# PaullyMac/routest

Measured on AMD Instinct MI355X. Metric: ETA preds/sec (whole node) + p50 /predict latency, 3-layer MLP bf16, higher is better.
Workload: dtype bf16

## Files before the change

### csrc/cch_bindings.cpp

```cpp
#include <torch/extension.h>
#include <ATen/hip/impl/HIPStreamMasqueradingAsCUDA.h>
#include <c10/core/DeviceGuard.h>

#include <chrono>
#include <cmath>
#include <memory>
#include <mutex>
#include <unordered_map>

#include "cch_gpu.h"
#include "ops.h"

namespace py = pybind11;

namespace {

#define CCH_CHECK_HIP(expr)                                                            \
  do {                                                                                 \
    hipError_t _e = (expr);                                                            \
    TORCH_CHECK(_e == hipSuccess, "HIP error in ", #expr, ": ", hipGetErrorString(_e)); \
  } while (0)

hipStream_t stream_of(int dev) { return c10::hip::getCurrentHIPStreamMasqueradingAsCUDA(dev).stream(); }

// ... 123 lines not shown
    d["async_pending"] = a.pending;
    d["async_build_ms"] = a.build_ms;
    d["async_alloc_ms"] = a.alloc_ms;
    d["async_hostcopy_ms"] = a.hostcopy_ms;
    d["builder_max_wg"] = g_->builder_pacing();
    d["async_paced"] = a.paced;
    return d;
  }

  void request_build(int64_t weather, int64_t congestion, int64_t weekhour, double age, bool urgent,
                     c10::optional<torch::Tensor> avoid, int64_t avoid_digest) {
    TORCH_CHECK(g_->has_eta(), "CchGpu: set_eta first");
    const rt::CchContext c = context(weather, congestion, weekhour, age, avoid, avoid_digest);
    g_->request_build(c, urgent);
  }
  bool is_cached(int64_t key) {
    std::shared_ptr<rt::CchMetricDev> m;
    return g_->cached_metric((uint64_t)key, m);
  }
  void set_cache_gb(double gb) { g_->set_cache_gb(gb); }
  void set_builder_pacing(int n, bool always) { g_->set_builder_pacing(n, always); }
  void set_unpack_serial(bool on) { g_->set_unpack_serial(on); }
  bool unpack_serial() const { return g_->unpack_serial(); }

  py::dict info(const rt::CchMetricDev& m, bool fresh) const {
    py::dict d;
    d["key"] = m.key;
    d["fresh"] = fresh;
    d["cost_ms"] = m.cost_ms;
    d["customize_ms"] = m.customize_ms;
    d["basic_ms"] = m.basic_ms;
    d["perfect_ms"] = m.perfect_ms;
    d["prune_ms"] = m.prune_ms;
    d["kept_f"] = m.kept_f;
    d["kept_b"] = m.kept_b;
    return d;
  }

  py::dict metric_for(int64_t weather, int64_t congestion, int64_t weekhour, double age, bool pin,
                      c10::optional<torch::Tensor> avoid, int64_t avoid_digest) {
    TORCH_CHECK(g_->has_eta(), "CchGpu: set_eta first");
    const rt::CchContext c = context(weather, congestion, weekhour, age, avoid, avoid_digest);
    const c10::DeviceGuard guard(c10::Device(c10::DeviceType::CUDA, dev_));
    std::shared_ptr<rt::CchMetricDev> m;
    bool fresh = false;
    hipError_t e;
// ... 98 lines not shown
    o.path = want_path ? path.data_ptr<int>() : nullptr;
    o.max_path = (int)max_path;
    const c10::DeviceGuard guard(src.device());
    std::lock_guard<std::mutex> lk(mu_);
    CCH_CHECK_HIP(g_->route(*m, src.data_ptr<int>(), dst.data_ptr<int>(), (int)Q, o, *sc_, stream_of(dev_)));
    return py::make_tuple(sec, met, st, len, path);
  }

  py::tuple matrix(int64_t key, torch::Tensor pts, torch::Tensor npts) {
    auto m = get(key);
    TORCH_CHECK(pts.is_cuda() && npts.is_cuda() && pts.dim() == 2 && pts.scalar_type() == torch::kInt32 &&
                    npts.scalar_type() == torch::kInt32 && npts.numel() == pts.size(0) && pts.is_contiguous(),
                "pts int32 [R, NM], npts int32 [R] on the router's GPU");
    const int R = (int)pts.size(0), NM = (int)pts.size(1);
    auto of = torch::TensorOptions().dtype(torch::kFloat32).device(torch::kCUDA, dev_);
    auto sec = torch::empty({R, NM, NM}, of), met = torch::empty({R, NM, NM}, of);
    const c10::DeviceGuard guard(pts.device());
    std::lock_guard<std::mutex> lk(mu_);
    CCH_CHECK_HIP(g_->matrix(*m, pts.data_ptr<int>(), npts.data_ptr<int>(), R, NM, sec.data_ptr<float>(),
                             met.data_ptr<float>(), nullptr, *sc_, stream_of(dev_)));
    return py::make_tuple(sec, met);
  }

  py::tuple matrix_rect(int64_t key, torch::Tensor src, torch::Tensor nsrc, torch::Tensor dst, torch::Tensor ndst,
                        int64_t meet) {
    auto m = get(key);
    for (const torch::Tensor* t : {&src, &nsrc, &dst, &ndst})
      TORCH_CHECK(t->is_cuda() && t->device().index() == dev_ && t->scalar_type() == torch::kInt32 && t->is_contiguous(),
                  "src / nsrc / dst / ndst: int32 on the router's GPU");
    TORCH_CHECK(src.dim() == 2 && dst.dim() == 2 && dst.size(0) == src.size(0) && nsrc.numel() == src.size(0) &&
                    ndst.numel() == src.size(0),
                "src [R, SM], dst [R, DM], nsrc [R], ndst [R]");
    const int64_t R = src.size(0), SM = src.size(1), DM = dst.size(1);
    TORCH_CHECK(R * (SM + DM) <= INT32_MAX && R * SM * DM <= INT32_MAX, "matrix_rect: too many chains or cells for one call");
    auto of = torch::TensorOptions().dtype(torch::kFloat32).device(torch::kCUDA, dev_);
    auto sec = torch::empty({R, SM, DM}, of), met = torch::empty({R, SM, DM}, of);
    const c10::DeviceGuard guard(src.device());
    std::lock_guard<std::mutex> lk(mu_);
    CCH_CHECK_HIP(g_->matrix_rect(*m, src.data_ptr<int>(), nsrc.data_ptr<int>(), dst.data_ptr<int>(),
                                  ndst.data_ptr<int>(), (int)R, (int)SM, (int)DM, sec.data_ptr<float>(),
                                  met.data_ptr<float>(), *sc_, stream_of(dev_), (int)meet));
    return py::make_tuple(sec, met);
  }

  py::tuple matrix_keep(int64_t key, torch::Tensor pts, torch::Tensor npts) {
    auto sm = matrix(key, pts, npts);
// ... 107 lines not shown

}

void bind_cch_gpu(py::module& m) {
  py::class_<PyCchGpu>(m, "CchGpu")
      .def(py::init<torch::Tensor, torch::Tensor, torch::Tensor, torch::Tensor, torch::Tensor, torch::Tensor,
                    torch::Tensor, int64_t>(),
           py::arg("indptr"), py::arg("indices"), py::arg("lat"), py::arg("lon"), py::arg("length"),
           py::arg("road_class"), py::arg("base_traffic"), py::arg("device"))
      .def("set_eta", &PyCchGpu::set_eta, py::arg("blob"), py::arg("H"), py::arg("norm"), py::arg("variant") = -1)
      .def("stats", &PyCchGpu::stats)
      .def("metric_for", &PyCchGpu::metric_for, py::arg("weather"), py::arg("congestion"), py::arg("weekhour"),
           py::arg("driver_age") = 35.0, py::arg("pin") = false, py::arg("avoid") = py::none(),
           py::arg("avoid_digest") = 0)
      .def("avoid_mask", &PyCchGpu::avoid_mask, py::arg("blob"))
      .def("unpin", &PyCchGpu::unpin, py::arg("key"))
      .def("pinned", &PyCchGpu::pinned)
      .def("metric_from_costs", &PyCchGpu::metric_from_costs, py::arg("key"), py::arg("cost"))
      .def("costs", &PyCchGpu::costs, py::arg("key"))
      .def("metric_dump", &PyCchGpu::metric_dump, py::arg("key"))
      .def("route", &PyCchGpu::route, py::arg("key"), py::arg("src"), py::arg("dst"), py::arg("max_path") = 4096,
           py::arg("want_path") = true)
      .def("matrix", &PyCchGpu::matrix, py::arg("key"), py::arg("pts"), py::arg("npts"))
      .def("matrix_rect", &PyCchGpu::matrix_rect, py::arg("key"), py::arg("src"), py::arg("nsrc"), py::arg("dst"),
           py::arg("ndst"), py::arg("meet") = 0)
      .def("matrix_keep", &PyCchGpu::matrix_keep, py::arg("key"), py::arg("pts"), py::arg("npts"))
      .def("legs_from_matrix", &PyCchGpu::legs_from_matrix, py::arg("key"), py::arg("tag"), py::arg("pts"), py::arg("r"),
           py::arg("i"), py::arg("j"), py::arg("max_path") = 4096, py::arg("want_path") = true)
      .def("one_to_all", &PyCchGpu::one_to_all, py::arg("key"), py::arg("src"), py::arg("reverse") = false,
           py::arg("fuse") = -1)
      .def("set_capacity", &PyCchGpu::set_capacity)
      .def("set_cache_gb", &PyCchGpu::set_cache_gb, py::arg("gb"))
      .def("set_builder_pacing", &PyCchGpu::set_builder_pacing, py::arg("max_workgroups"), py::arg("always") = false)
      .def("set_unpack_serial", &PyCchGpu::set_unpack_serial, py::arg("on"))
      .def("unpack_serial", &PyCchGpu::unpack_serial)
      .def("request_build", &PyCchGpu::request_build, py::arg("weather"), py::arg("congestion"), py::arg("weekhour"),
           py::arg("driver_age") = 35.0, py::arg("urgent") = true, py::arg("avoid") = py::none(),
           py::arg("avoid_digest") = 0)
      .def("is_cached", &PyCchGpu::is_cached, py::arg("key"))
      .def("ptr", &PyCchGpu::ptr)
      .def("topology_arrays", &PyCchGpu::topology_arrays);
}
```

### csrc/cch_gpu.h

```cpp
#pragma once
#include <hip/hip_runtime.h>

#include <cstdint>
#include <cstdlib>
#include <cstring>
#include <atomic>
#include <chrono>
#include <condition_variable>
#include <deque>
#include <functional>
#include <list>
#include <memory>
#include <mutex>
#include <thread>
#include <unordered_set>
#include <vector>

#include "common.h"
#include "runtime/cch.h"

namespace rt {

struct CchContext {
  int weather = 2, congestion = 1, weekhour = 9;
// ... 15 lines not shown
  float* len_up = nullptr;
  float* len_dn = nullptr;
  int32_t* cnt_up = nullptr;
  int32_t* cnt_dn = nullptr;
  int32_t* f_ptr = nullptr;
  int32_t* b_ptr = nullptr;
  int4* f_rec = nullptr;
  int4* b_rec = nullptr;
  int64_t kept_f = 0, kept_b = 0;
  double customize_ms = 0.0, cost_ms = 0.0;
  double basic_ms = 0.0, perfect_ms = 0.0, prune_ms = 0.0;
  double alloc_ms = 0.0, hostcopy_ms = 0.0;
  std::vector<float> host_cost;
  std::shared_ptr<const std::vector<int32_t>> avoid;
  ~CchMetricDev();
};

struct CchScratch {
  float* dist = nullptr;
  int32_t* pred = nullptr;
  int32_t* node = nullptr;
  size_t jobs_cap = 0;
  int32_t* jobs = nullptr;
  int32_t* arcs = nullptr;
  int32_t* narcs = nullptr;
  size_t pairs_cap = 0;
  int32_t* pj = nullptr;
  size_t pj_cap = 0;
  uint64_t chain_tag = 0;
  int chain_nm = 0, chain_r = 0;
  int device = 0;
  std::vector<void*> old;
  ~CchScratch();
  hipError_t ensure(size_t jobs, size_t pairs, int stride, int max_arcs);
};

struct CchAllScratch {
  float* sec = nullptr;
  float* met = nullptr;
  size_t blocks_cap = 0;
  int device = 0;
  std::vector<void*> old;
  ~CchAllScratch();
  hipError_t ensure(size_t blocks, size_t N);
};

// ... 75 lines not shown
  double cache_gb() { std::lock_guard<std::mutex> lk(mu_); return cache_gb_; }
  int capacity() { std::lock_guard<std::mutex> lk(mu_); return capacity_; }
  int64_t metric_bytes() const { return metric_bytes_.load(); }
  int cached() { std::lock_guard<std::mutex> lk(mu_); return (int)cache_.size(); }

  void request_build(const CchContext& c, bool urgent = true);
  void start_builders();
  int add_build_listener(std::function<void(uint64_t, bool)> cb);
  void remove_build_listener(int id);
  struct AsyncStats {
    long long queued = 0, built = 0, failed = 0;
    int pending = 0;
    double build_ms = 0.0, alloc_ms = 0.0, hostcopy_ms = 0.0;
    long long paced = 0;
  };
  AsyncStats async_stats();
  void set_builder_pacing(int n, bool always = false) {
    builder_max_wg_.store(n < 0 ? 0 : n);
    pace_always_.store(always);
  }
  int builder_pacing() const { return builder_max_wg_.load(); }
  void set_unpack_serial(bool on) { unpack_serial_.store(on); }
  bool unpack_serial() const { return unpack_serial_.load(); }
  void note_queries() {
    query_us_.store(std::chrono::duration_cast<std::chrono::microseconds>(
                        std::chrono::steady_clock::now().time_since_epoch()).count(),
                    std::memory_order_relaxed);
  }
  bool serving_now() const {
    const long long now = std::chrono::duration_cast<std::chrono::microseconds>(
                              std::chrono::steady_clock::now().time_since_epoch()).count();
    return now - query_us_.load(std::memory_order_relaxed) < 250000;
  }

  hipError_t route(const CchMetricDev& m, const int* d_src, const int* d_dst, int Q, const CchRouteOut& o,
                   CchScratch& sc, hipStream_t s);
  hipError_t matrix(const CchMetricDev& m, const int* d_pts, const int* d_npts, int R, int NM, float* d_sec,
                    float* d_met, double* d_D64, CchScratch& sc, hipStream_t s);
  hipError_t legs_from_matrix(const CchMetricDev& m, const int* d_src, const int* d_r, const int* d_i, const int* d_j,
                              int Q, uint64_t tag, const CchRouteOut& o, CchScratch& sc, hipStream_t s);
  static constexpr int MAX_ARCS = 1024;
  enum { MEET_AUTO = 0, MEET_RECT = 1, MEET_PAIRS = 2, MEET_NONE = 3 };
  hipError_t matrix_rect(const CchMetricDev& m, const int* d_src, const int* d_nsrc, const int* d_dst,
                         const int* d_ndst, int R, int SM, int DM, float* d_sec, float* d_met, CchScratch& sc,
                         hipStream_t s, int meet = MEET_AUTO);

// ... 1 lines not shown
                        CchAllScratch& sc, hipStream_t s, int fuse = -1);
  static constexpr size_t ALL_SCRATCH_BYTES = 1ull << 30;
  static constexpr int ALL_FUSE_WIDTH = 4;

  static CchMView view(const CchMetricDev& m) {
    return CchMView{m.f_ptr, m.b_ptr, m.f_rec, m.b_rec, m.len_up, m.len_dn, m.sub_up, m.sub_dn, m.cnt_up, m.cnt_dn};
  }
  hipError_t route_multi(const CchMView* d_mv, const int* d_grp, const int* d_src, const int* d_dst, int Q,
                         const CchRouteOut& o, CchScratch& sc, hipStream_t s);
  hipError_t matrix_multi(const CchMView* d_mv, const int* d_row_grp, const int* d_pts, const int* d_npts, int R, int NM,
                          float* d_sec, float* d_met, double* d_D64, CchScratch& sc, hipStream_t s);
  hipError_t legs_from_matrix_multi(const CchMView* d_mv, const int* d_grp, const int* d_src, const int* d_r,
                                    const int* d_i, const int* d_j, int Q, uint64_t tag, const CchRouteOut& o,
                                    CchScratch& sc, hipStream_t s);

 private:
  hipError_t route_impl(const CchMetricDev* m, const CchMView* mv, const int* grp, const int* d_src, const int* d_dst,
                        int Q, const CchRouteOut& o, CchScratch& sc, hipStream_t s);
  hipError_t matrix_impl(const CchMetricDev* m, const CchMView* mv, const int* grp, const int* d_pts, const int* d_npts,
                         int R, int NM, float* d_sec, float* d_met, double* d_D64, CchScratch& sc, hipStream_t s);
  hipError_t legs_impl(const CchMetricDev* m, const CchMView* mv, const int* grp, const int* d_src, const int* d_r,
                       const int* d_i, const int* d_j, int Q, uint64_t tag, const CchRouteOut& o, CchScratch& sc,
                       hipStream_t s);
  hipError_t launch_unpack(const CchMetricDev* m, const CchMView* mv, const int* grp, int Q, const int* d_src,
                           CchScratch& sc, const CchRouteOut& o, hipStream_t s);
  rcch::Topology T_;
  int dev_ = 0;
  int32_t *d_up_ptr = nullptr, *d_up_head = nullptr, *d_arc_lo = nullptr, *d_parent = nullptr, *d_depth = nullptr;
  int32_t *d_rank = nullptr, *d_node = nullptr, *d_edge_arc = nullptr;
  uint8_t* d_edge_dir = nullptr;
  float* d_length = nullptr;
  uint8_t *d_class = nullptr, *d_base_traffic = nullptr;
  int32_t *d_hnodes = nullptr, *d_dnodes = nullptr;
  int32_t* d_dlev_ptr = nullptr;
  int64_t *d_bofs = nullptr, *d_pofs = nullptr;
  std::vector<int64_t> bofs_, pofs_, aofs_;
  std::vector<int> plev_kmax_;
  bool accel_ = false;
  void build_tables();
  void free_tables();
  bool build_triangles(const std::vector<int64_t>& tofs);
  int32_t* d_tri = nullptr;
  int64_t n_tri = 0;
  bool build_tasks(const std::vector<int64_t>& tofs);
  bool build_pull_records(const std::vector<int64_t>& tofs);
  void* d_btask = nullptr;
// ... 51 lines not shown
  int32_t *d_esrc = nullptr, *d_edst = nullptr, *d_qx = nullptr, *d_qy = nullptr;
  std::atomic<uint64_t> tag_ctr_{0};
  void builder_loop(int idx);
  void start_builders_locked();
  void notify_built(uint64_t key, bool ok);
  std::vector<std::thread> bths_;
  std::mutex bmu_;
  std::condition_variable bcv_;
  std::deque<CchContext> bq_;
  std::unordered_set<uint64_t> bpending_;
  bool bstop_ = false;
  std::mutex lmu_;
  std::vector<std::pair<int, std::function<void(uint64_t, bool)>>> listeners_;
  int next_listener_ = 1;
  std::atomic<long long> n_bqueued_{0}, n_bbuilt_{0}, n_bfailed_{0};
  std::atomic<long long> us_build_{0}, us_alloc_{0}, us_hostcopy_{0};
  std::atomic<long long> query_us_{-(1LL << 40)};
  std::atomic<bool> pace_always_{false};
  std::atomic<long long> n_paced_{0};
  std::atomic<int> builder_max_wg_{[] {
    const char* v = std::getenv("ROUTEST_CCH_BUILDER_MAX_WG");
    return v ? std::max(0, std::atoi(v)) : -1;
  }()};
  std::atomic<bool> unpack_serial_{[] {
    const char* v = std::getenv("ROUTEST_CCH_UNPACK");
    return v != nullptr && std::strcmp(v, "serial") == 0;
  }()};
};

}
```

### csrc/cch_query.hip

```cpp
#include "cch_dev.h"
#include "cch_gpu.h"

namespace rt {

using namespace cchd;

namespace {

constexpr int SWEEP_AHEAD = 3;
constexpr int SWEEP_RECS = 4;

typedef int sweep_v4i __attribute__((ext_vector_type(4)));

struct SweepRecs {
  sweep_v4i r[SWEEP_RECS];
};

__device__ __forceinline__ SweepRecs sweep_fetch(const int4* __restrict__ rec, int pb, int pe, int i, int L, int lane) {
  SweepRecs v;
  const int ii = i < 63 ? i : 63;
  const int b = __shfl(pb, ii);
  const int e = i < L ? __shfl(pe, ii) : b;
#pragma unroll
  for (int k = 0; k < SWEEP_RECS; ++k) {
    const int idx = b + lane + 64 * k;
    const int4* p = rec + (idx < e ? idx : 0);
    asm volatile("global_load_dwordx4 %0, %1, off" : "=v"(v.r[k]) : "v"(p));
  }
  return v;
}

template <int NEWER>
__device__ __forceinline__ void sweep_wait(SweepRecs& q) {
  static_assert(NEWER * SWEEP_RECS <= 63, "vmcnt range");
  asm volatile("s_waitcnt vmcnt(%4)" : "+v"(q.r[0]), "+v"(q.r[1]), "+v"(q.r[2]), "+v"(q.r[3]) : "n"(NEWER * SWEEP_RECS));
}

__device__ __forceinline__ void sweep_relax(float* sd, int32_t* sp, float dx, int w, int hd, int arc) {
  const float nd = dx + __int_as_float(w);
  if (nd < sd[hd]) {
    sd[hd] = nd;
    sp[hd] = arc;
  }
}

__global__ __launch_bounds__(64) void sweep_kernel(const int32_t* __restrict__ jobs, int J,
                                                   const int32_t* __restrict__ parent,
                                                   const int32_t* __restrict__ depth, int N,
                                                   const int32_t* __restrict__ f_ptr, const int4* __restrict__ f_rec,
                                                   const int32_t* __restrict__ b_ptr, const int4* __restrict__ b_rec,
                                                   int stride, float* __restrict__ out_dist,
                                                   int32_t* __restrict__ out_pred, int32_t* __restrict__ out_node,
                                                   const CchMView* __restrict__ mv, const int32_t* __restrict__ grp,
                                                   int gdiv) {
  extern __shared__ unsigned char smem[];
  float* sd = reinterpret_cast<float*>(smem);
  int32_t* sp = reinterpret_cast<int32_t*>(smem + (size_t)stride * 4);
  const int j = blockIdx.x;
  if (j >= J) return;
  const int lane = threadIdx.x;
  const int code = jobs[j];
  if (code < 0) return;
  const int r = code >> 1;
  const bool fwd = (code & 1) == 0;
  if (mv != nullptr) {
    const CchMView& v = mv[grp[j / gdiv]];
    f_ptr = v.f_ptr;
    f_rec = v.f_rec;
    b_ptr = v.b_ptr;
    b_rec = v.b_rec;
  }
  const int32_t* __restrict__ ptr = fwd ? f_ptr : b_ptr;
  const int4* __restrict__ rec = fwd ? f_rec : b_rec;
  const int D = depth[r];
  for (int d = lane; d <= D; d += 64) {
    sd[d] = F_INF;
    sp[d] = -1;
  }
  __syncthreads();
  if (lane == 0) sd[D] = 0.f;
  __syncthreads();
  const size_t base = (size_t)j * stride;
// ... 42 lines not shown
      sweep_wait<3>(qc);
      node(i + 2, qc);
      qc = sweep_fetch(rec, pb, pe, i + 6, L, lane);
      sweep_wait<3>(qd);
      node(i + 3, qd);
    }
    sweep_wait<0>(qa);
    sweep_wait<0>(qb);
    sweep_wait<0>(qc);
    x = next;
    d -= L;
    cand = ncand;
    par = npar;
    pb = npb;
    pe = npe;
  }
  __syncthreads();
  for (int dd = lane; dd <= D; dd += 64) {
    out_dist[base + dd] = sd[dd];
    out_pred[base + dd] = sp[dd];
  }
}

__global__ __launch_bounds__(64) void meet_kernel(int P, const int32_t* __restrict__ pjf, const int32_t* __restrict__ pjb,
                                                  int jf0, int jb0, const int32_t* __restrict__ jobs, int stride,
                                                  const float* __restrict__ sdist, const int32_t* __restrict__ spred,
                                                  const int32_t* __restrict__ snode, const int32_t* __restrict__ depth,
                                                  const int32_t* __restrict__ arc_lo, const float* __restrict__ len_up,
                                                  const float* __restrict__ len_dn, float* __restrict__ out_sec,
                                                  float* __restrict__ out_met, int* __restrict__ out_status,
                                                  int32_t* __restrict__ arcs, int32_t* __restrict__ narcs, int max_arcs,
                                                  const CchMView* __restrict__ mv, const int32_t* __restrict__ grp,
                                                  int gdiv) {
  __shared__ int32_t fw[4096];
  const int q = blockIdx.x;
  if (q >= P) return;
  const int lane = threadIdx.x;
  if (mv != nullptr) {
    const CchMView& v = mv[grp[q / gdiv]];
    len_up = v.len_up;
    len_dn = v.len_dn;
  }
  const int jf = pjf ? pjf[q] : jf0 + 2 * q;
  const int jb = pjb ? pjb[q] : jb0 + 2 * q;
  if (jobs[jf] < 0 || jobs[jb] < 0) {
    if (threadIdx.x == 0) {
      if (out_sec) out_sec[q] = -1.f;
      if (out_met) out_met[q] = -1.f;
      if (out_status) out_status[q] = 1;
      if (narcs) narcs[q] = 0;
    }
    return;
  }
  const int s = jobs[jf] >> 1, t = jobs[jb] >> 1;
  const int ds = depth[s], dt = depth[t];
  const size_t bf = (size_t)jf * stride, bb = (size_t)jb * stride;
  int status = 1;
// ... 13 lines not shown
        best = v;
        bestd = d;
      }
    }
#pragma unroll
    for (int o = 32; o >= 1; o >>= 1) {
      const float ov = __shfl_xor(best, o);
      const int od = __shfl_xor(bestd, o);
      if (ov < best || (ov == best && od > bestd)) {
        best = ov;
        bestd = od;
      }
    }
    if (best < F_INF) status = 0;
  }
  if (lane != 0) return;
  float met = 0.f;
  int n = 0;
  if (status == 0) {
    int nf = 0;
    for (int slot = bestd; slot != ds;) {
      const int a = spred[bf + slot];
      met += len_up[a];
      if (nf < 4096) fw[nf] = a;
      ++nf;
      slot = depth[arc_lo[a]];
    }
    if (arcs != nullptr) {
      int32_t* out = arcs + (size_t)q * max_arcs;
      if (nf > 4096 || nf > max_arcs) status = 4;
      for (int i = nf - 1; i >= 0 && status == 0; --i) out[n++] = fw[i] << 1;
      for (int slot = bestd; slot != dt && status == 0;) {
        const int a = spred[bb + slot];
        met += len_dn[a];
        if (n >= max_arcs) { status = 4; break; }
        out[n++] = (a << 1) | 1;
        slot = depth[arc_lo[a]];
      }
    } else {
      for (int slot = bestd; slot != dt;) {
        const int a = spred[bb + slot];
        met += len_dn[a];
        slot = depth[arc_lo[a]];
      }
    }
  }
  if (out_sec) out_sec[q] = status == 0 ? best : -1.f;
  if (out_met) out_met[q] = status == 0 ? met : -1.f;
  if (out_status) out_status[q] = status;
  if (narcs) narcs[q] = n;
}

constexpr int UNPACK_STACK = 128;
// ... 390 lines not shown
  const int rem = (int)(g % ((long long)SM * DM));
  const int i = rem / DM, j = rem % DM;
  float s = sec[g], m = met[g];
  const size_t jrow = (size_t)r * (SM + DM);
  if (i >= nsrc[r] || j >= ndst[r] || (jobs[jrow + i] >> 1) == (jobs[jrow + SM + j] >> 1)) s = m = 0.f;
  else {
    if (s < 0.f) s = F_INF;
    if (m < 0.f) m = F_INF;
  }
  sec[g] = s;
  met[g] = m;
}

}

CchScratch::~CchScratch() {
  int cur = 0;
  (void)hipGetDevice(&cur);
  (void)hipSetDevice(device);
  dfree(dist);
  dfree(pred);
  dfree(node);
  dfree(jobs);
  dfree(arcs);
  dfree(narcs);
  dfree(pj);
  for (void* p : old) (void)hipFree(p);
  (void)hipSetDevice(cur);
}

hipError_t CchScratch::ensure(size_t J, size_t P, int stride, int max_arcs) {
  hipError_t e = hipSuccess;
  auto retire = [&](auto*& p) {
    if (p) old.push_back((void*)p);
    p = nullptr;
  };
  if (J > jobs_cap) {
    retire(dist);
    retire(pred);
    retire(node);
    retire(jobs);
    const size_t cap = std::max(J, jobs_cap * 3 / 2);
    if ((e = dmalloc(dist, cap * stride)) != hipSuccess) return e;
    if ((e = dmalloc(pred, cap * stride)) != hipSuccess) return e;
    if ((e = dmalloc(node, cap * stride)) != hipSuccess) return e;
    if ((e = dmalloc(jobs, cap)) != hipSuccess) return e;
    jobs_cap = cap;
  }
  if (P > pairs_cap) {
    retire(arcs);
    retire(narcs);
    const size_t cap = std::max(P, pairs_cap * 3 / 2);
    if ((e = dmalloc(arcs, cap * (size_t)max_arcs)) != hipSuccess) return e;
    if ((e = dmalloc(narcs, cap)) != hipSuccess) return e;
    pairs_cap = cap;
  }
  return e;
}

hipError_t CchGpu::launch_unpack(const CchMetricDev* m, const CchMView* mv, const int* grp, int Q, const int* d_src,
                                 CchScratch& sc, const CchRouteOut& o, hipStream_t s) {
  const bool serial_only = unpack_serial();
  const int32_t* sub_up = m ? m->sub_up : nullptr;
  const int32_t* sub_dn = m ? m->sub_dn : nullptr;
  if (!serial_only) {
    constexpr int G = 64 / UNPACK_LANES;
    hipLaunchKernelGGL(unpack_coop_kernel, dim3((Q + G - 1) / G), dim3(64), 0, s, Q, d_src, sc.arcs, sc.narcs, MAX_ARCS,
                       sub_up, sub_dn, m ? m->cnt_up : nullptr, m ? m->cnt_dn : nullptr, d_arc_lo, d_up_head, d_node,
                       o.status, o.len, o.path, o.max_path, o.edges, mv, grp);
    hipError_t e = hipGetLastError();
    if (e != hipSuccess) return e;
  }
  hipLaunchKernelGGL(unpack_kernel, dim3(blocks_for(Q, 64)), dim3(64), 0, s, Q, d_src, sc.arcs, sc.narcs, MAX_ARCS,
                     sub_up, sub_dn, d_arc_lo, d_up_head, d_node, o.status, o.len, o.path, o.max_path,
                     serial_only ? -1 : UNPACK_MAX_ARCS, o.edges, mv, grp);
  return hipGetLastError();
}

hipError_t CchGpu::route_impl(const CchMetricDev* m, const CchMView* mv, const int* grp, const int* d_src,
                              const int* d_dst, int Q, const CchRouteOut& o, CchScratch& sc, hipStream_t s) {
  if (Q <= 0) return hipSuccess;
  const int S = stride();
  sc.device = dev_;
  sc.chain_tag = 0;
  hipError_t e = sc.ensure((size_t)2 * Q, (size_t)Q, S, MAX_ARCS);
  if (e != hipSuccess) return e;
  hipLaunchKernelGGL(route_jobs_kernel, dim3(blocks_for(Q, 256)), dim3(256), 0, s, d_src, d_dst, Q, d_rank, T_.N,
                     sc.jobs);
  hipLaunchKernelGGL(sweep_kernel, dim3(2 * Q), dim3(64), (size_t)S * 8, s, sc.jobs, 2 * Q, d_parent, d_depth, T_.N,
                     m ? m->f_ptr : nullptr, m ? m->f_rec : nullptr, m ? m->b_ptr : nullptr, m ? m->b_rec : nullptr, S,
                     sc.dist, sc.pred, sc.node, mv, grp, 2);
  if ((e = hipGetLastError()) != hipSuccess) return e;
  hipLaunchKernelGGL(meet_kernel, dim3(Q), dim3(64), 0, s, Q, nullptr, nullptr, 0, 1, sc.jobs, S, sc.dist, sc.pred,
                     sc.node, d_depth, d_arc_lo, m ? m->len_up : nullptr, m ? m->len_dn : nullptr, o.sec, o.metres,
                     o.status, o.path ? sc.arcs : nullptr, o.path ? sc.narcs : nullptr, MAX_ARCS, mv, grp, 1);
  if ((e = hipGetLastError()) != hipSuccess) return e;
  if (o.path != nullptr) e = launch_unpack(m, mv, grp, Q, d_src, sc, o, s);
  return e;
}

hipError_t CchGpu::route(const CchMetricDev& m, const int* d_src, const int* d_dst, int Q, const CchRouteOut& o,
                         CchScratch& sc, hipStream_t s) {
  return route_impl(&m, nullptr, nullptr, d_src, d_dst, Q, o, sc, s);
}

hipError_t CchGpu::route_multi(const CchMView* d_mv, const int* d_grp, const int* d_src, const int* d_dst, int Q,
                               const CchRouteOut& o, CchScratch& sc, hipStream_t s) {
  if (d_mv == nullptr || d_grp == nullptr) return hipErrorInvalidValue;
  return route_impl(nullptr, d_mv, d_grp, d_src, d_dst, Q, o, sc, s);
}

hipError_t CchGpu::matrix_impl(const CchMetricDev* m, const CchMView* mv, const int* grp, const int* d_pts,
                               const int* d_npts, int R, int NM, float* d_sec, float* d_met, double* d_D64,
                               CchScratch& sc, hipStream_t s) {
  if (R <= 0 || NM <= 0) return hipSuccess;
  if (d_sec == nullptr || d_met == nullptr) return hipErrorInvalidValue;
  const int S = stride();
  sc.device = dev_;
  const size_t J = (size_t)R * NM * 2, P = (size_t)R * NM * NM;
  hipError_t e = sc.ensure(J, (P * 2 + MAX_ARCS - 1) / MAX_ARCS + 1, S, MAX_ARCS);
  if (e != hipSuccess) return e;
  int32_t* pjf = sc.arcs;
  int32_t* pjb = sc.arcs + P;
  float* sec = d_sec;
  float* met = d_met;
  hipLaunchKernelGGL(matrix_jobs_kernel, dim3(blocks_for((long long)R * NM, 256)), dim3(256), 0, s, d_pts, d_npts, R, NM,
                     d_rank, T_.N, sc.jobs);
  hipLaunchKernelGGL(matrix_pairs_kernel, dim3(blocks_for((long long)P, 256)), dim3(256), 0, s, d_npts, R, NM, pjf, pjb);
  hipLaunchKernelGGL(sweep_kernel, dim3((unsigned)J), dim3(64), (size_t)S * 8, s, sc.jobs, (int)J, d_parent, d_depth,
                     T_.N, m ? m->f_ptr : nullptr, m ? m->f_rec : nullptr, m ? m->b_ptr : nullptr,
                     m ? m->b_rec : nullptr, S, sc.dist, sc.pred, sc.node, mv, grp, 2 * NM);
  if ((e = hipGetLastError()) != hipSuccess) return e;
  hipLaunchKernelGGL(meet_kernel, dim3((unsigned)P), dim3(64), 0, s, (int)P, pjf, pjb, 0, 0, sc.jobs, S, sc.dist,
                     sc.pred, sc.node, d_depth, d_arc_lo, m ? m->len_up : nullptr, m ? m->len_dn : nullptr, sec, met,
                     nullptr, nullptr, nullptr, MAX_ARCS, mv, grp, NM * NM);
  if ((e = hipGetLastError()) != hipSuccess) return e;
  hipLaunchKernelGGL(matrix_out_kernel, dim3(blocks_for((long long)P, 256)), dim3(256), 0, s, d_npts, R, NM, sec, met,
                     d_D64);
  e = hipGetLastError();
  sc.chain_tag = e == hipSuccess ? ++tag_ctr_ : 0;
  sc.chain_nm = NM;
  sc.chain_r = R;
  return e;
}

hipError_t CchGpu::matrix(const CchMetricDev& m, const int* d_pts, const int* d_npts, int R, int NM, float* d_sec,
                          float* d_met, double* d_D64, CchScratch& sc, hipStream_t s) {
  return matrix_impl(&m, nullptr, nullptr, d_pts, d_npts, R, NM, d_sec, d_met, d_D64, sc, s);
}

hipError_t CchGpu::matrix_multi(const CchMView* d_mv, const int* d_row_grp, const int* d_pts, const int* d_npts, int R,
                                int NM, float* d_sec, float* d_met, double* d_D64, CchScratch& sc, hipStream_t s) {
  if (d_mv == nullptr || d_row_grp == nullptr) return hipErrorInvalidValue;
  return matrix_impl(nullptr, d_mv, d_row_grp, d_pts, d_npts, R, NM, d_sec, d_met, d_D64, sc, s);
}

hipError_t CchGpu::matrix_rect(const CchMetricDev& m, const int* d_src, const int* d_nsrc, const int* d_dst,
                               const int* d_ndst, int R, int SM, int DM, float* d_sec, float* d_met, CchScratch& sc,
                               hipStream_t s, int meet) {
  if (R <= 0 || SM <= 0 || DM <= 0) return hipSuccess;
  if (d_sec == nullptr || d_met == nullptr || meet < MEET_AUTO || meet > MEET_NONE) return hipErrorInvalidValue;
  const int S = stride();
  const size_t J = (size_t)R * ((size_t)SM + DM), P = (size_t)R * SM * DM;
  if (J > (size_t)INT32_MAX || P > (size_t)INT32_MAX) return hipErrorInvalidValue;
  const size_t lds = (size_t)S * 12;
  const bool fits = lds + MEET_TILE * 8 <= 64 * 1024;
  if (meet == MEET_RECT && !fits) return hipErrorInvalidValue;
  if (meet == MEET_AUTO) meet = fits ? MEET_RECT : MEET_PAIRS;
  sc.device = dev_;
  sc.chain_tag = 0;
  hipError_t e = sc.ensure(J, meet == MEET_PAIRS ? (P * 2 + MAX_ARCS - 1) / MAX_ARCS + 1 : 0, S, MAX_ARCS);
  if (e != hipSuccess) return e;
  hipLaunchKernelGGL(rect_jobs_kernel, dim3(blocks_for((long long)J, 256)), dim3(256), 0, s, d_src, d_nsrc, d_dst,
                     d_ndst, R, SM, DM, d_rank, T_.N, sc.jobs);
  hipLaunchKernelGGL(sweep_kernel, dim3((unsigned)J), dim3(64), (size_t)S * 8, s, sc.jobs, (int)J, d_parent, d_depth,
                     T_.N, m.f_ptr, m.f_rec, m.b_ptr, m.b_rec, S, sc.dist, sc.pred, sc.node, nullptr, nullptr, 1);
  if ((e = hipGetLastError()) != hipSuccess) return e;
  if (meet == MEET_RECT) {
    const size_t blocks = (size_t)R * SM * ((DM + MEET_TILE - 1) / MEET_TILE);
    hipLaunchKernelGGL(meet_rect_kernel, dim3((unsigned)blocks), dim3(MEET_THREADS), lds, s, SM, DM, d_nsrc, d_ndst,
                       sc.jobs, S, sc.dist, sc.pred, sc.node, d_depth, d_arc_lo, m.len_up, m.len_dn, d_sec, d_met);
  } else if (meet == MEET_PAIRS) {
    int32_t* pjf = sc.arcs;
    int32_t* pjb = sc.arcs + P;
    hipLaunchKernelGGL(rect_pairs_kernel, dim3(blocks_for((long long)P, 256)), dim3(256), 0, s, R, SM, DM, pjf, pjb);
    hipLaunchKernelGGL(meet_kernel, dim3((unsigned)P), dim3(64), 0, s, (int)P, pjf, pjb, 0, 0, sc.jobs, S, sc.dist,
                       sc.pred, sc.node, d_depth, d_arc_lo, m.len_up, m.len_dn, d_sec, d_met, nullptr, nullptr, nullptr,
                       MAX_ARCS, nullptr, nullptr, 1);
    if ((e = hipGetLastError()) != hipSuccess) return e;
    hipLaunchKernelGGL(rect_out_kernel, dim3(blocks_for((long long)P, 256)), dim3(256), 0, s, d_nsrc, d_ndst, R, SM, DM,
                       sc.jobs, d_sec, d_met);
  }
  return hipGetLastError();
}

hipError_t CchGpu::legs_impl(const CchMetricDev* m, const CchMView* mv, const int* grp, const int* d_src,
                             const int* d_r, const int* d_i, const int* d_j, int Q, uint64_t tag, const CchRouteOut& o,
                             CchScratch& sc, hipStream_t s) {
  if (Q <= 0) return hipSuccess;
  if (tag == 0 || tag != sc.chain_tag) return hipErrorInvalidValue;
  const int S = stride();
  hipError_t e = sc.ensure(0, (size_t)Q, S, MAX_ARCS);
  if (e != hipSuccess) return e;
  if ((size_t)Q > sc.pj_cap) {
    if (sc.pj) sc.old.push_back((void*)sc.pj);
    sc.pj = nullptr;
    const size_t cap = std::max((size_t)Q, sc.pj_cap * 3 / 2);
    if ((e = dmalloc(sc.pj, 2 * cap)) != hipSuccess) return e;
    sc.pj_cap = cap;
  }
  int32_t* pjf = sc.pj;
  int32_t* pjb = sc.pj + sc.pj_cap;
  hipLaunchKernelGGL(leg_pairs_kernel, dim3(blocks_for(Q, 256)), dim3(256), 0, s, sc.chain_nm, d_r, d_i, d_j, Q,
                     sc.chain_r, pjf, pjb);
  if ((e = hipGetLastError()) != hipSuccess) return e;
  hipLaunchKernelGGL(meet_kernel, dim3(Q), dim3(64), 0, s, Q, pjf, pjb, 0, 0, sc.jobs, S, sc.dist, sc.pred, sc.node,
                     d_depth, d_arc_lo, m ? m->len_up : nullptr, m ? m->len_dn : nullptr, o.sec, o.metres, o.status,
                     o.path ? sc.arcs : nullptr, o.path ? sc.narcs : nullptr, MAX_ARCS, mv, grp, 1);
  if ((e = hipGetLastError()) != hipSuccess) return e;
  if (o.path != nullptr) e = launch_unpack(m, mv, grp, Q, d_src, sc, o, s);
  return e;
}

hipError_t CchGpu::legs_from_matrix(const CchMetricDev& m, const int* d_src, const int* d_r, const int* d_i,
                                    const int* d_j, int Q, uint64_t tag, const CchRouteOut& o, CchScratch& sc,
                                    hipStream_t s) {
  return legs_impl(&m, nullptr, nullptr, d_src, d_r, d_i, d_j, Q, tag, o, sc, s);
}

hipError_t CchGpu::legs_from_matrix_multi(const CchMView* d_mv, const int* d_grp, const int* d_src, const int* d_r,
                                          const int* d_i, const int* d_j, int Q, uint64_t tag, const CchRouteOut& o,
                                          CchScratch& sc, hipStream_t s) {
  if (d_mv == nullptr || d_grp == nullptr) return hipErrorInvalidValue;
  return legs_impl(nullptr, d_mv, d_grp, d_src, d_r, d_i, d_j, Q, tag, o, sc, s);
}

}
```

Before: 6.751 billion.

## Sort sweep jobs by code, interleave placement, and template meet kernel on arcs

Before the CCH sweep, jobs are radix-sorted by their code so that related queries are grouped, invalid jobs are dropped, and work is spread in an 8-way interleave across workgroups (on by default via an env var). The meet kernel is templated so variants that skip path arcs no longer reserve 16KB of LDS, which can raise occupancy. Python bindings are also added for multi-metric routing and matrix calls. This costs an extra iota launch, a radix sort and a count kernel per sweep, plus more scratch memory.

```diff
diff --git a/csrc/cch_bindings.cpp b/csrc/cch_bindings.cpp
--- a/csrc/cch_bindings.cpp
+++ b/csrc/cch_bindings.cpp
@@ -169,6 +169,8 @@
   void set_builder_pacing(int n, bool always) { g_->set_builder_pacing(n, always); }
   void set_unpack_serial(bool on) { g_->set_unpack_serial(on); }
   bool unpack_serial() const { return g_->unpack_serial(); }
+  void set_sweep_place(bool on) { g_->set_sweep_place(on); }
+  bool sweep_place() const { return g_->sweep_place(); }
 
   py::dict info(const rt::CchMetricDev& m, bool fresh) const {
     py::dict d;
@@ -313,6 +315,80 @@
     return py::make_tuple(sec, met);
   }
 
+  torch::Tensor views_of(const std::vector<int64_t>& keys, std::vector<std::shared_ptr<rt::CchMetricDev>>& hold) {
+    TORCH_CHECK(!keys.empty(), "keys: at least one metric");
+    std::vector<rt::CchMView> mv;
+    for (int64_t k : keys) {
+      hold.push_back(get(k));
+      mv.push_back(rt::CchGpu::view(*hold.back()));
+    }
+    const int64_t bytes = (int64_t)(mv.size() * sizeof(rt::CchMView));
+    auto h = torch::empty({bytes}, torch::TensorOptions().dtype(torch::kUInt8));
+    std::memcpy(h.data_ptr(), mv.data(), (size_t)bytes);
+    return h.to(torch::Device(torch::kCUDA, dev_));
+  }
+  void check_grp(const torch::Tensor& grp, int64_t n, size_t G) {
+    TORCH_CHECK(grp.is_cuda() && grp.device().index() == dev_ && grp.scalar_type() == torch::kInt32 &&
+                    grp.is_contiguous() && grp.numel() == n,
+                "grp: int32 on the router's GPU, one entry per pair / request row");
+    if (n > 0) TORCH_CHECK(grp.min().item<int>() >= 0 && grp.max().item<int>() < (int)G, "grp out of range");
+  }
+
+  py::tuple route_multi(std::vector<int64_t> keys, torch::Tensor grp, torch::Tensor src, torch::Tensor dst,
+                        int64_t max_path, bool want_path) {
+    std::vector<std::shared_ptr<rt::CchMetricDev>> hold;
+    auto mv = views_of(keys, hold);
+    TORCH_CHECK(src.is_cuda() && dst.is_cuda() && src.device().index() == dev_ && dst.device().index() == dev_ &&
+                    src.scalar_type() == torch::kInt32 && dst.scalar_type() == torch::kInt32 &&
+                    src.is_contiguous() && dst.is_contiguous() && src.numel() == dst.numel(),
+                "src/dst: int32 [Q] on the router's GPU");
+    const int64_t Q = src.numel();
+    check_grp(grp, Q, keys.size());
+    const int N = g_->topo().N;
+    if (Q > 0) {
+      const auto mn = torch::minimum(src.min(), dst.min()).item<int>();
+      const auto mx = torch::maximum(src.max(), dst.max()).item<int>();
+      TORCH_CHECK(mn >= 0 && mx < N, "node id out of range");
+    }
+    auto o32 = torch::TensorOptions().dtype(torch::kInt32).device(torch::kCUDA, dev_);
+    auto of = torch::TensorOptions().dtype(torch::kFloat32).device(torch::kCUDA, dev_);
+    auto sec = torch::empty({Q}, of), met = torch::empty({Q}, of);
+    auto st = torch::empty({Q}, o32), len = torch::zeros({Q}, o32);
+    auto path = want_path ? torch::empty({Q, max_path}, o32) : torch::empty({0, max_path}, o32);
+    rt::CchRouteOut o;
+    o.sec = sec.data_ptr<float>();
+    o.metres = met.data_ptr<float>();
+    o.status = st.data_ptr<int>();
+    o.len = len.data_ptr<int>();
+    o.path = want_path ? path.data_ptr<int>() : nullptr;
+    o.max_path = (int)max_path;
+    const c10::DeviceGuard guard(src.device());
+    std::lock_guard<std::mutex> lk(mu_);
+    CCH_CHECK_HIP(g_->route_multi(reinterpret_cast<const rt::CchMView*>(mv.data_ptr()), grp.data_ptr<int>(),
+                                  src.data_ptr<int>(), dst.data_ptr<int>(), (int)Q, o, *sc_, stream_of(dev_)));
+    CCH_CHECK_HIP(hipStreamSynchronize(stream_of(dev_)));
+    return py::make_tuple(sec, met, st, len, path);
+  }
+
+  py::tuple matrix_multi(std::vector<int64_t> keys, torch::Tensor row_grp, torch::Tensor pts, torch::Tensor npts) {
+    std::vector<std::shared_ptr<rt::CchMetricDev>> hold;
+    auto mv = views_of(keys, hold);
+    TORCH_CHECK(pts.is_cuda() && npts.is_cuda() && pts.dim() == 2 && pts.scalar_type() == torch::kInt32 &&
+                    npts.scalar_type() == torch::kInt32 && npts.numel() == pts.size(0) && pts.is_contiguous(),
+                "pts int32 [R, NM], npts int32 [R] on the router's GPU");
+    const int R = (int)pts.size(0), NM = (int)pts.size(1);
+    check_grp(row_grp, R, keys.size());
+    auto of = torch::TensorOptions().dtype(torch::kFloat32).device(torch::kCUDA, dev_);
+    auto sec = torch::empty({R, NM, NM}, of), met = torch::empty({R, NM, NM}, of);
+    const c10::DeviceGuard guard(pts.device());
+    std::lock_guard<std::mutex> lk(mu_);
+    CCH_CHECK_HIP(g_->matrix_multi(reinterpret_cast<const rt::CchMView*>(mv.data_ptr()), row_grp.data_ptr<int>(),
+                                   pts.data_ptr<int>(), npts.data_ptr<int>(), R, NM, sec.data_ptr<float>(),
+                                   met.data_ptr<float>(), nullptr, *sc_, stream_of(dev_)));
+    CCH_CHECK_HIP(hipStreamSynchronize(stream_of(dev_)));
+    return py::make_tuple(sec, met);
+  }
+
   py::tuple matrix_rect(int64_t key, torch::Tensor src, torch::Tensor nsrc, torch::Tensor dst, torch::Tensor ndst,
                         int64_t meet) {
     auto m = get(key);
@@ -466,6 +542,10 @@
       .def("route", &PyCchGpu::route, py::arg("key"), py::arg("src"), py::arg("dst"), py::arg("max_path") = 4096,
            py::arg("want_path") = true)
       .def("matrix", &PyCchGpu::matrix, py::arg("key"), py::arg("pts"), py::arg("npts"))
+      .def("route_multi", &PyCchGpu::route_multi, py::arg("keys"), py::arg("grp"), py::arg("src"), py::arg("dst"),
+           py::arg("max_path") = 4096, py::arg("want_path") = true)
+      .def("matrix_multi", &PyCchGpu::matrix_multi, py::arg("keys"), py::arg("row_grp"), py::arg("pts"),
+           py::arg("npts"))
       .def("matrix_rect", &PyCchGpu::matrix_rect, py::arg("key"), py::arg("src"), py::arg("nsrc"), py::arg("dst"),
            py::arg("ndst"), py::arg("meet") = 0)
       .def("matrix_keep", &PyCchGpu::matrix_keep, py::arg("key"), py::arg("pts"), py::arg("npts"))
@@ -478,6 +558,8 @@
       .def("set_builder_pacing", &PyCchGpu::set_builder_pacing, py::arg("max_workgroups"), py::arg("always") = false)
       .def("set_unpack_serial", &PyCchGpu::set_unpack_serial, py::arg("on"))
       .def("unpack_serial", &PyCchGpu::unpack_serial)
+      .def("set_sweep_place", &PyCchGpu::set_sweep_place, py::arg("on"))
+      .def("sweep_place", &PyCchGpu::sweep_place)
       .def("request_build", &PyCchGpu::request_build, py::arg("weather"), py::arg("congestion"), py::arg("weekhour"),
            py::arg("driver_age") = 35.0, py::arg("urgent") = true, py::arg("avoid") = py::none(),
            py::arg("avoid_digest") = 0)
diff --git a/csrc/cch_gpu.h b/csrc/cch_gpu.h
--- a/csrc/cch_gpu.h
+++ b/csrc/cch_gpu.h
@@ -61,6 +61,12 @@
   int32_t* node = nullptr;
   size_t jobs_cap = 0;
   int32_t* jobs = nullptr;
+  int32_t* perm = nullptr;
+  int32_t* iota = nullptr;
+  uint32_t* skeys = nullptr;
+  int32_t* nreal = nullptr;
+  void* sort_tmp = nullptr;
+  size_t sort_bytes = 0;
   int32_t* arcs = nullptr;
   int32_t* narcs = nullptr;
   size_t pairs_cap = 0;
@@ -182,6 +188,8 @@
   int builder_pacing() const { return builder_max_wg_.load(); }
   void set_unpack_serial(bool on) { unpack_serial_.store(on); }
   bool unpack_serial() const { return unpack_serial_.load(); }
+  void set_sweep_place(bool on) { sweep_place_.store(on); }
+  bool sweep_place() const { return sweep_place_.load(); }
   void note_queries() {
     query_us_.store(std::chrono::duration_cast<std::chrono::microseconds>(
                         std::chrono::steady_clock::now().time_since_epoch()).count(),
@@ -229,6 +237,12 @@
   hipError_t legs_impl(const CchMetricDev* m, const CchMView* mv, const int* grp, const int* d_src, const int* d_r,
                        const int* d_i, const int* d_j, int Q, uint64_t tag, const CchRouteOut& o, CchScratch& sc,
                        hipStream_t s);
+  hipError_t place_jobs(CchScratch& sc, size_t J, hipStream_t s);
+  hipError_t launch_sweep(const CchMetricDev* m, const CchMView* mv, const int* grp, int gdiv, size_t J,
+                          CchScratch& sc, hipStream_t s);
+  void launch_meet(bool want_arcs, int P, const int32_t* pjf, const int32_t* pjb, int jf0, int jb0, int S,
+                   const CchMetricDev* m, const CchMView* mv, const int* grp, int gdiv, float* sec, float* met,
+                   int* status, CchScratch& sc, hipStream_t s);
   hipError_t launch_unpack(const CchMetricDev* m, const CchMView* mv, const int* grp, int Q, const int* d_src,
                            CchScratch& sc, const CchRouteOut& o, hipStream_t s);
   rcch::Topology T_;
@@ -326,6 +340,10 @@
     const char* v = std::getenv("ROUTEST_CCH_BUILDER_MAX_WG");
     return v ? std::max(0, std::atoi(v)) : -1;
   }()};
+  std::atomic<bool> sweep_place_{[] {
+    const char* v = std::getenv("ROUTEST_CCH_SWEEP_PLACE");
+    return v == nullptr || std::strcmp(v, "0") != 0;
+  }()};
   std::atomic<bool> unpack_serial_{[] {
     const char* v = std::getenv("ROUTEST_CCH_UNPACK");
     return v != nullptr && std::strcmp(v, "serial") == 0;
diff --git a/csrc/cch_query.hip b/csrc/cch_query.hip
--- a/csrc/cch_query.hip
+++ b/csrc/cch_query.hip
@@ -1,3 +1,5 @@
+#include <hipcub/hipcub.hpp>
+
 #include "cch_dev.h"
 #include "cch_gpu.h"
 
@@ -45,6 +47,7 @@
 }
 
 __global__ __launch_bounds__(64) void sweep_kernel(const int32_t* __restrict__ jobs, int J,
+                                                   const int32_t* __restrict__ perm, const int32_t* __restrict__ nreal,
                                                    const int32_t* __restrict__ parent,
                                                    const int32_t* __restrict__ depth, int N,
                                                    const int32_t* __restrict__ f_ptr, const int4* __restrict__ f_rec,
@@ -56,8 +59,15 @@
   extern __shared__ unsigned char smem[];
   float* sd = reinterpret_cast<float*>(smem);
   int32_t* sp = reinterpret_cast<int32_t*>(smem + (size_t)stride * 4);
-  const int j = blockIdx.x;
-  if (j >= J) return;
+  int j = blockIdx.x;
+  if (perm != nullptr) {
+    const int jr = min(nreal[0], J);
+    const int per = (jr + 7) >> 3;
+    const int pos = (j & 7) * per + (j >> 3);
+    if ((j >> 3) >= per || pos >= jr) return;
+    j = perm[pos];
+  }
+  if (j < 0 || j >= J) return;
   const int lane = threadIdx.x;
   const int code = jobs[j];
   if (code < 0) return;
@@ -146,6 +156,7 @@
   }
 }
 
+template <bool ARCS>
 __global__ __launch_bounds__(64) void meet_kernel(int P, const int32_t* __restrict__ pjf, const int32_t* __restrict__ pjb,
                                                   int jf0, int jb0, const int32_t* __restrict__ jobs, int stride,
                                                   const float* __restrict__ sdist, const int32_t* __restrict__ spred,
@@ -156,7 +167,8 @@
                                                   int32_t* __restrict__ arcs, int32_t* __restrict__ narcs, int max_arcs,
                                                   const CchMView* __restrict__ mv, const int32_t* __restrict__ grp,
                                                   int gdiv) {
-  __shared__ int32_t fw[4096];
+  constexpr int FW = ARCS ? CchGpu::MAX_ARCS : 1;
+  __shared__ int32_t fw[FW];
   const int q = blockIdx.x;
   if (q >= P) return;
   const int lane = threadIdx.x;
@@ -216,13 +228,13 @@
     for (int slot = bestd; slot != ds;) {
       const int a = spred[bf + slot];
       met += len_up[a];
-      if (nf < 4096) fw[nf] = a;
+      if (ARCS && nf < FW) fw[nf] = a;
       ++nf;
       slot = depth[arc_lo[a]];
     }
-    if (arcs != nullptr) {
+    if (ARCS) {
       int32_t* out = arcs + (size_t)q * max_arcs;
-      if (nf > 4096 || nf > max_arcs) status = 4;
+      if (nf > FW || nf > max_arcs) status = 4;
       for (int i = nf - 1; i >= 0 && status == 0; --i) out[n++] = fw[i] << 1;
       for (int slot = bestd; slot != dt && status == 0;) {
         const int a = spred[bb + slot];
@@ -659,6 +671,11 @@
   dfree(pred);
   dfree(node);
   dfree(jobs);
+  dfree(perm);
+  dfree(iota);
+  dfree(skeys);
+  dfree(nreal);
+  if (sort_tmp) (void)hipFree(sort_tmp);
   dfree(arcs);
   dfree(narcs);
   dfree(pj);
@@ -677,11 +694,26 @@
     retire(pred);
     retire(node);
     retire(jobs);
+    retire(perm);
+    retire(iota);
+    retire(skeys);
+    retire(sort_tmp);
     const size_t cap = std::max(J, jobs_cap * 3 / 2);
+    jobs_cap = 0;
+    sort_bytes = 0;
+    if (cap > (size_t)INT32_MAX) return hipErrorInvalidValue;
     if ((e = dmalloc(dist, cap * stride)) != hipSuccess) return e;
     if ((e = dmalloc(pred, cap * stride)) != hipSuccess) return e;
     if ((e = dmalloc(node, cap * stride)) != hipSuccess) return e;
     if ((e = dmalloc(jobs, cap)) != hipSuccess) return e;
+    if ((e = dmalloc(perm, cap)) != hipSuccess) return e;
+    if ((e = dmalloc(iota, cap)) != hipSuccess) return e;
+    if ((e = dmalloc(skeys, cap)) != hipSuccess) return e;
+    if (nreal == nullptr && (e = dmalloc(nreal, 1)) != hipSuccess) return e;
+    size_t tb = 0;
+    if ((e = hipcub::DeviceRadixSort::SortPairs(nullptr, tb, skeys, skeys, iota, perm, (int)cap)) != hipSuccess) return e;
+    if ((e = hipMalloc(&sort_tmp, std::max<size_t>(tb, 16))) != hipSuccess) return e;
+    sort_bytes = tb;
     jobs_cap = cap;
   }
   if (P > pairs_cap) {
@@ -693,6 +725,66 @@
     pairs_cap = cap;
   }
   return e;
+}
+
+namespace {
+
+__global__ void place_iota_kernel(int J, int32_t* __restrict__ iota) {
+  const int i = blockIdx.x * blockDim.x + threadIdx.x;
+  if (i < J) iota[i] = i;
+}
+
+__global__ void place_count_kernel(const uint32_t* __restrict__ keys, int J, int32_t* __restrict__ nreal) {
+  const int i = blockIdx.x * blockDim.x + threadIdx.x;
+  if (i >= J) return;
+  const bool real = (int32_t)keys[i] >= 0;
+  if (i == 0 && !real) nreal[0] = 0;
+  if (real && (i == J - 1 || (int32_t)keys[i + 1] < 0)) nreal[0] = i + 1;
+}
+
+}
+
+hipError_t CchGpu::place_jobs(CchScratch& sc, size_t J, hipStream_t s) {
+  if (J == 0 || J > sc.jobs_cap || J > (size_t)INT32_MAX) return hipErrorInvalidValue;
+  hipLaunchKernelGGL(place_iota_kernel, dim3(blocks_for((long long)J, 256)), dim3(256), 0, s, (int)J, sc.iota);
+  hipError_t e = hipGetLastError();
+  if (e != hipSuccess) return e;
+  size_t tb = sc.sort_bytes;
+  e = hipcub::DeviceRadixSort::SortPairs(sc.sort_tmp, tb, reinterpret_cast<const uint32_t*>(sc.jobs), sc.skeys,
+                                         sc.iota, sc.perm, (int)J, 0, 32, s);
+  if (e != hipSuccess) return e;
+  hipLaunchKernelGGL(place_count_kernel, dim3(blocks_for((long long)J, 256)), dim3(256), 0, s, sc.skeys, (int)J,
+                     sc.nreal);
+  return hipGetLastError();
+}
+
+void CchGpu::launch_meet(bool want_arcs, int P, const int32_t* pjf, const int32_t* pjb, int jf0, int jb0, int S,
+                         const CchMetricDev* m, const CchMView* mv, const int* grp, int gdiv, float* sec, float* met,
+                         int* status, CchScratch& sc, hipStream_t s) {
+  const float* len_up = m ? m->len_up : nullptr;
+  const float* len_dn = m ? m->len_dn : nullptr;
+  if (want_arcs)
+    hipLaunchKernelGGL(meet_kernel<true>, dim3((unsigned)P), dim3(64), 0, s, P, pjf, pjb, jf0, jb0, sc.jobs, S, sc.dist,
+                       sc.pred, sc.node, d_depth, d_arc_lo, len_up, len_dn, sec, met, status, sc.arcs, sc.narcs,
+                       MAX_ARCS, mv, grp, gdiv);
+  else
+    hipLaunchKernelGGL(meet_kernel<false>, dim3((unsigned)P), dim3(64), 0, s, P, pjf, pjb, jf0, jb0, sc.jobs, S,
+                       sc.dist, sc.pred, sc.node, d_depth, d_arc_lo, len_up, len_dn, sec, met, status, nullptr,
+                       nullptr, MAX_ARCS, mv, grp, gdiv);
+}
+
+hipError_t CchGpu::launch_sweep(const CchMetricDev* m, const CchMView* mv, const int* grp, int gdiv, size_t J,
+                                CchScratch& sc, hipStream_t s) {
+  const int S = stride();
+  const bool place = sweep_place();
+  hipError_t e = hipSuccess;
+  if (place && (e = place_jobs(sc, J, s)) != hipSuccess) return e;
+  const size_t grid = place ? (J + 7) / 8 * 8 : J;
+  hipLaunchKernelGGL(sweep_kernel, dim3((unsigned)grid), dim3(64), (size_t)S * 8, s, sc.jobs, (int)J,
+                     place ? sc.perm : nullptr, sc.nreal, d_parent, d_depth, T_.N, m ? m->f_ptr : nullptr,
+                     m ? m->f_rec : nullptr, m ? m->b_ptr : nullptr, m ? m->b_rec : nullptr, S, sc.dist, sc.pred,
+                     sc.node, mv, grp, gdiv);
+  return hipGetLastError();
 }
 
 hipError_t CchGpu::launch_unpack(const CchMetricDev* m, const CchMView* mv, const int* grp, int Q, const int* d_src,
@@ -724,13 +816,8 @@
   if (e != hipSuccess) return e;
   hipLaunchKernelGGL(route_jobs_kernel, dim3(blocks_for(Q, 256)), dim3(256), 0, s, d_src, d_dst, Q, d_rank, T_.N,
                      sc.jobs);
-  hipLaunchKernelGGL(sweep_kernel, dim3(2 * Q), dim3(64), (size_t)S * 8, s, sc.jobs, 2 * Q, d_parent, d_depth, T_.N,
-                     m ? m->f_ptr : nullptr, m ? m->f_rec : nullptr, m ? m->b_ptr : nullptr, m ? m->b_rec : nullptr, S,
-                     sc.dist, sc.pred, sc.node, mv, grp, 2);
-  if ((e = hipGetLastError()) != hipSuccess) return e;
-  hipLaunchKernelGGL(meet_kernel, dim3(Q), dim3(64), 0, s, Q, nullptr, nullptr, 0, 1, sc.jobs, S, sc.dist, sc.pred,
-                     sc.node, d_depth, d_arc_lo, m ? m->len_up : nullptr, m ? m->len_dn : nullptr, o.sec, o.metres,
-                     o.status, o.path ? sc.arcs : nullptr, o.path ? sc.narcs : nullptr, MAX_ARCS, mv, grp, 1);
+  if ((e = launch_sweep(m, mv, grp, 2, (size_t)2 * Q, sc, s)) != hipSuccess) return e;
+  launch_meet(o.path != nullptr, Q, nullptr, nullptr, 0, 1, S, m, mv, grp, 1, o.sec, o.metres, o.status, sc, s);
   if ((e = hipGetLastError()) != hipSuccess) return e;
   if (o.path != nullptr) e = launch_unpack(m, mv, grp, Q, d_src, sc, o, s);
   return e;
@@ -764,13 +851,8 @@
   hipLaunchKernelGGL(matrix_jobs_kernel, dim3(blocks_for((long long)R * NM, 256)), dim3(256), 0, s, d_pts, d_npts, R, NM,
                      d_rank, T_.N, sc.jobs);
   hipLaunchKernelGGL(matrix_pairs_kernel, dim3(blocks_for((long long)P, 256)), dim3(256), 0, s, d_npts, R, NM, pjf, pjb);
-  hipLaunchKernelGGL(sweep_kernel, dim3((unsigned)J), dim3(64), (size_t)S * 8, s, sc.jobs, (int)J, d_parent, d_depth,
-                     T_.N, m ? m->f_ptr : nullptr, m ? m->f_rec : nullptr, m ? m->b_ptr : nullptr,
-                     m ? m->b_rec : nullptr, S, sc.dist, sc.pred, sc.node, mv, grp, 2 * NM);
-  if ((e = hipGetLastError()) != hipSuccess) return e;
-  hipLaunchKernelGGL(meet_kernel, dim3((unsigned)P), dim3(64), 0, s, (int)P, pjf, pjb, 0, 0, sc.jobs, S, sc.dist,
-                     sc.pred, sc.node, d_depth, d_arc_lo, m ? m->len_up : nullptr, m ? m->len_dn : nullptr, sec, met,
-                     nullptr, nullptr, nullptr, MAX_ARCS, mv, grp, NM * NM);
+  if ((e = launch_sweep(m, mv, grp, 2 * NM, J, sc, s)) != hipSuccess) return e;
+  launch_meet(false, (int)P, pjf, pjb, 0, 0, S, m, mv, grp, NM * NM, sec, met, nullptr, sc, s);
   if ((e = hipGetLastError()) != hipSuccess) return e;
   hipLaunchKernelGGL(matrix_out_kernel, dim3(blocks_for((long long)P, 256)), dim3(256), 0, s, d_npts, R, NM, sec, met,
                      d_D64);
@@ -810,9 +892,7 @@
   if (e != hipSuccess) return e;
   hipLaunchKernelGGL(rect_jobs_kernel, dim3(blocks_for((long long)J, 256)), dim3(256), 0, s, d_src, d_nsrc, d_dst,
                      d_ndst, R, SM, DM, d_rank, T_.N, sc.jobs);
-  hipLaunchKernelGGL(sweep_kernel, dim3((unsigned)J), dim3(64), (size_t)S * 8, s, sc.jobs, (int)J, d_parent, d_depth,
-                     T_.N, m.f_ptr, m.f_rec, m.b_ptr, m.b_rec, S, sc.dist, sc.pred, sc.node, nullptr, nullptr, 1);
-  if ((e = hipGetLastError()) != hipSuccess) return e;
+  if ((e = launch_sweep(&m, nullptr, nullptr, 1, J, sc, s)) != hipSuccess) return e;
   if (meet == MEET_RECT) {
     const size_t blocks = (size_t)R * SM * ((DM + MEET_TILE - 1) / MEET_TILE);
     hipLaunchKernelGGL(meet_rect_kernel, dim3((unsigned)blocks), dim3(MEET_THREADS), lds, s, SM, DM, d_nsrc, d_ndst,
@@ -821,9 +901,7 @@
     int32_t* pjf = sc.arcs;
     int32_t* pjb = sc.arcs + P;
     hipLaunchKernelGGL(rect_pairs_kernel, dim3(blocks_for((long long)P, 256)), dim3(256), 0, s, R, SM, DM, pjf, pjb);
-    hipLaunchKernelGGL(meet_kernel, dim3((unsigned)P), dim3(64), 0, s, (int)P, pjf, pjb, 0, 0, sc.jobs, S, sc.dist,
-                       sc.pred, sc.node, d_depth, d_arc_lo, m.len_up, m.len_dn, d_sec, d_met, nullptr, nullptr, nullptr,
-                       MAX_ARCS, nullptr, nullptr, 1);
+    launch_meet(false, (int)P, pjf, pjb, 0, 0, S, &m, nullptr, nullptr, 1, d_sec, d_met, nullptr, sc, s);
     if ((e = hipGetLastError()) != hipSuccess) return e;
     hipLaunchKernelGGL(rect_out_kernel, dim3(blocks_for((long long)P, 256)), dim3(256), 0, s, d_nsrc, d_ndst, R, SM, DM,
                        sc.jobs, d_sec, d_met);
@@ -851,9 +929,7 @@
   hipLaunchKernelGGL(leg_pairs_kernel, dim3(blocks_for(Q, 256)), dim3(256), 0, s, sc.chain_nm, d_r, d_i, d_j, Q,
                      sc.chain_r, pjf, pjb);
   if ((e = hipGetLastError()) != hipSuccess) return e;
-  hipLaunchKernelGGL(meet_kernel, dim3(Q), dim3(64), 0, s, Q, pjf, pjb, 0, 0, sc.jobs, S, sc.dist, sc.pred, sc.node,
-                     d_depth, d_arc_lo, m ? m->len_up : nullptr, m ? m->len_dn : nullptr, o.sec, o.metres, o.status,
-                     o.path ? sc.arcs : nullptr, o.path ? sc.narcs : nullptr, MAX_ARCS, mv, grp, 1);
+  launch_meet(o.path != nullptr, Q, pjf, pjb, 0, 0, S, m, mv, grp, 1, o.sec, o.metres, o.status, sc, s);
   if ((e = hipGetLastError()) != hipSuccess) return e;
   if (o.path != nullptr) e = launch_unpack(m, mv, grp, Q, d_src, sc, o, s);
   return e;
```

Result: no change. 6.766 billion (median of 3 runs) (+0.2%).
